# radiusxyz/delay-encryption-in-halo2

Measured on AMD Instinct MI355X. Metric: pallas_msm_mpoints_per_s_at_2^20, higher is better.
Workload: dtype u256; 1 GPU; 1 x MSM(2^20, pallas) + 1 x NTT(2^20, pasta_fp) per step per GPU, uniform scalars, SRS tables resident; configs_index=1, steps_in_flight=4, parallelism=single GPU, attempts=1

## Files before the change

delay-encryption-in-halo2_amd/csrc/msm.cuh:

```cuda
#pragma once
#include <algorithm>
#include <cstdlib>
#include <cstdio>
#include <vector>

#include "ec29.cuh"
#include "internal.hpp"
#include "msm_plan.hpp"

#ifndef MSM_ACC_WAVES_ATTR
#ifdef MSM_ACC_CAP
#define MSM_ACC_WAVES_ATTR __attribute__((amdgpu_waves_per_eu(MSM_ACC_CAP, MSM_ACC_CAP)))
#else
#define MSM_ACC_WAVES_ATTR __attribute__((amdgpu_waves_per_eu(4, 4)))
#endif
#endif
#ifdef MSM_HIST_VGPR64
#define MSM_HIST_ATTR __attribute__((amdgpu_num_vgpr(64)))
#else
#define MSM_HIST_ATTR
#endif

#ifndef MSM_TAIL_PRIO
#define MSM_TAIL_PRIO 0
#endif
FP_DEV void msm_tail_prio() {
#if MSM_TAIL_PRIO > 0
    __builtin_amdgcn_s_setprio(MSM_TAIL_PRIO);
#endif
}

FP_DEV u32 merge2_class(u32 S) { return S <= 2 ? 0u : S <= 4 ? 1u : S <= 8 ? 2u : S <= 64 ? 3u : S <= MERGE2_CHUNK ? 4u : 5u; }

FP_DEV bool fe_is_zero_words(const fe& a) { return (a.v[0] | a.v[1] | a.v[2] | a.v[3] | a.v[4] | a.v[5] | a.v[6] | a.v[7]) == 0; }

template <class FS, class Fn>
FP_DEV void for_each_digit(const fe& mont_scalar, u32 c, u32 w_lo, u32 w_hi, Fn f) {
    if (fe_is_zero_words(mont_scalar)) return;
    fe s = f_from_mont<FS>(mont_scalar);
    u32 bits = 0;
#pragma unroll
    for (int i = 0; i < 8; i++) if (s.v[i]) bits = 32u * i + (32u - (u32)__clz((int)s.v[i]));
    const u32 w_end = min(w_hi, (bits + c - 1) / c + 1);
    const u32 mask = (1u << c) - 1, halfv = 1u << (c - 1);
    u32 carry = 0;
    for (u32 w = 0; w < w_end; w++) {
        u32 raw = (s.v[0] & mask) + carry;
#pragma unroll
        for (int i = 0; i < 7; i++) s.v[i] = (s.v[i] >> c) | (s.v[i + 1] << (32 - c));
        s.v[7] >>= c;
        bool neg = raw > halfv;
        carry = neg ? 1u : 0u;
        u32 mag = neg ? (1u << c) - raw : raw;
        if (mag != 0 && w >= w_lo) f(w, mag - 1, neg);
    }
}

struct DigitStream {
    fe s;
    u32 carry, c, mask, halfv;
    template <class FS>
    FP_DEV void init(const fe& mont_scalar, u32 c_) {
        s = f_from_mont<FS>(mont_scalar);
        c = c_; mask = (1u << c) - 1; halfv = 1u << (c - 1); carry = 0;
    }
    FP_DEV bool exhausted() const { return carry == 0 && fe_is_zero_words(s); }
    FP_DEV void next(u32& bucket, bool& neg) {
        u32 raw = (s.v[0] & mask) + carry;
#pragma unroll
        for (int i = 0; i < 7; i++) s.v[i] = (s.v[i] >> c) | (s.v[i + 1] << (32 - c));
        s.v[7] >>= c;
        neg = raw > halfv;
        carry = neg ? 1u : 0u;
        u32 mag = neg ? (1u << c) - raw : raw;
        bucket = mag - 1;
    }
};

FP_DEV bool wave_value_groups(const fe& s, bool active, u32 lane, u32 max_groups, u32& leader, u32& cnt, u32& rank) {
    unsigned long long rem = __ballot(active);
    leader = lane; cnt = 1; rank = 0;
    for (u32 n = 0; rem; n++) {
        if (n == max_groups) return false;
        const int ld = __ffsll((long long)rem) - 1;
        bool eq = active;
#pragma unroll
        for (int w = 0; w < 8; w++) eq &= s.v[w] == (u32)__shfl((int)s.v[w], ld);
        const unsigned long long m = __ballot(eq);
        if (eq) { leader = (u32)ld; cnt = (u32)__popcll(m); rank = (u32)__popcll(m & ((1ull << lane) - 1)); }
        rem &= ~m;
    }
    return true;
}

template <class FS, bool PACK16>
__global__ __launch_bounds__(MSM_SORT_THREADS) MSM_HIST_ATTR void k_msm_hist(MsmGeom g, const fe* scalars, u32* bh, u32* pc) {
    msm_tail_prio();
    extern __shared__ u32 lhist[];
    const u32 bat = blockIdx.z;
    const u32 w_lo = g.G == 1 ? 0 : blockIdx.y * g.wb, w_hi = g.G == 1 ? g.W : min(g.W, w_lo + g.wb);
    const u32 ng = g.G == 1 ? 1 : w_hi - w_lo, grp0 = g.G == 1 ? 0 : w_lo;
    for (u32 b = threadIdx.x; b < (PACK16 ? ng * g.nb / 2 : ng * g.nb); b += blockDim.x) lhist[b] = 0;
    __syncthreads();
    const fe* sc = scalars + (u64)bat * g.n;
    const u32 per = (g.n + g.slices - 1) / g.slices;
    const u32 beg = blockIdx.x * per, end = min(beg + per, g.n);
    const bool one = g.G == 1;
    for (u32 i0 = beg + threadIdx.x; i0 < end; i0 += 4 * blockDim.x) {
        fe s4[4];
#pragma unroll
        for (int j = 0; j < 4; j++)
            if (i0 + j * blockDim.x < end) s4[j] = f_load(&sc[i0 + j * blockDim.x]);
#pragma unroll
        for (int j = 0; j < 4; j++) {
            const bool valid = i0 + j * blockDim.x < end;
            u32 gl, weight, grank;
            const bool grouped = wave_value_groups(s4[j], valid, threadIdx.x & 63, 4, gl, weight, grank);
            if (!grouped) weight = 1;
            const bool counts = grouped ? valid && (threadIdx.x & 63) == gl : valid;
            if (counts)
                for_each_digit<FS>(s4[j], g.c, w_lo, w_hi, [&](u32 w, u32 bucket, bool) {
                    const u32 slot = (one ? 0u : (w - w_lo) * g.nb) + bucket;
                    if (PACK16) atomicAdd(&lhist[slot >> 1], weight << ((slot & 1u) << 4));
                    else atomicAdd(&lhist[slot], weight);
                });
        }
    }
    __syncthreads();
    const u32 sub = msm_sub_bits(g.c), P = g.nb >> sub;
    for (u32 gi = 0; gi < ng; gi++) {
        const u64 gidx = (u64)bat * g.G + grp0 + gi;
        const u32* lh = lhist + (PACK16 ? gi * g.nb / 2 : gi * g.nb);
        if (PACK16) {
            u32* out = bh + ((gidx * g.slices + blockIdx.x) * g.nb) / 2;
            for (u32 w = threadIdx.x; w < g.nb / 2; w += blockDim.x) out[w] = lh[w];
        } else {
            u32* out = bh + (gidx * g.slices + blockIdx.x) * g.nb;
            for (u32 b = threadIdx.x; b < g.nb; b += blockDim.x) out[b] = lh[b];
        }
        u32* pout = pc + (gidx * g.slices + blockIdx.x) * P;
        const u32 nsub = 1u << sub, lane = threadIdx.x & 63;
        for (u32 q = threadIdx.x >> 6; q < P; q += blockDim.x >> 6) {
            u32 sum = 0;
            if (PACK16) {
                for (u32 w = lane; w < nsub / 2; w += 64) { const u32 x = lh[(q << sub) / 2 + w]; sum += (x & 0xffffu) + (x >> 16); }
            } else {
                for (u32 b = lane; b < nsub; b += 64) sum += lh[(q << sub) + b];
            }
#pragma unroll
            for (int d = 32; d > 0; d >>= 1) sum += __shfl_down(sum, d);
            if (lane == 0) pout[q] = sum;
        }
    }
}

template <bool SRC16>
FP_DEV u32 colscan_one(u32 nb, u32 slices, u32 total_buckets, u32* bh, const unsigned short* src16, u32* count, u32 gb) {
    if (gb >= total_buckets) return 0;
    u32 grp = gb / nb, b = gb - grp * nb;
    u32* col = bh + (u64)grp * slices * nb + b;
    const unsigned short* col16 = SRC16 ? src16 + (u64)grp * slices * nb + b : nullptr;
    u32 run = 0;
    u32 k = 0;
    for (; k + 16 <= slices; k += 16) {
        u32 v[16];
#pragma unroll
        for (int j = 0; j < 16; j++) v[j] = SRC16 ? (u32)col16[(u64)(k + j) * nb] : col[(u64)(k + j) * nb];
#pragma unroll
        for (int j = 0; j < 16; j++) {
            col[(u64)(k + j) * nb] = run;
            run += v[j];
        }
    }
    for (; k < slices; k++) {
        u32 v = SRC16 ? (u32)col16[(u64)k * nb] : col[(u64)k * nb];
        col[(u64)k * nb] = run;
        run += v;
    }
    if (count) count[gb] = run;
    return run;
}
static __global__ __launch_bounds__(SCAN_THREADS) void k_msm_colscan(u32 nb, u32 slices, u32 total_buckets, u32* bh, const unsigned short* bh16, u32* count, u32 blocks_a, u32 P,
                                                                     u32 total_parts, u32* pc, u32* bsum_items, u32* bsum_tasks, u32* merge_counters) {
    msm_tail_prio();
    if (blockIdx.x == 0 && threadIdx.x < MSM_MERGE_COUNTERS) merge_counters[threadIdx.x] = 0;
    if (blockIdx.x >= blocks_a) {
        colscan_one<false>(P, slices, total_parts, pc, nullptr, nullptr, (blockIdx.x - blocks_a) * blockDim.x + threadIdx.x);
        return;
    }
    const u32 gb0 = blockIdx.x * blockDim.x + threadIdx.x;
    const u32 v = bh16 ? colscan_one<true>(nb, slices, total_buckets, bh, bh16, count, gb0) : colscan_one<false>(nb, slices, total_buckets, bh, nullptr, count, gb0);
    u32 si = v, st = v ? 1u : 0u;
#pragma unroll
    for (int d = 32; d > 0; d >>= 1) { si += __shfl_down(si, d); st += __shfl_down(st, d); }
    __shared__ u32 w_i[SCAN_THREADS / 64], w_t[SCAN_THREADS / 64];
    if ((threadIdx.x & 63) == 0) { w_i[threadIdx.x >> 6] = si; w_t[threadIdx.x >> 6] = st; }
    __syncthreads();
    if (threadIdx.x == 0) {
        u32 a = 0, b = 0;
        for (u32 w = 0; w < SCAN_THREADS / 64; w++) { a += w_i[w]; b += w_t[w]; }
        bsum_items[blockIdx.x] = a; bsum_tasks[blockIdx.x] = b;
    }
}

static __global__ __launch_bounds__(SCAN_THREADS) void k_scan_offsets(const u32* cnt, u32 total, const u32* bsum_items, const u32* bsum_tasks, u32 nblocks, u32* geo, u32 resident,
                                                                      u32 lmax, u32 lcap, u32 kmin, u32* off, u32* nrank, u32* rbeg, u32* rend, u32* lists, u32 cap) {
    msm_tail_prio();
    __shared__ u32 s_i[SCAN_THREADS], s_t[SCAN_THREADS];
    __shared__ u32 w4[4][SCAN_THREADS / 64];
    const u32 tid = threadIdx.x, lane = tid & 63, wave = tid >> 6;
    u32 bi = 0, bt = 0, ti = 0;
    for (u32 j = tid; j < nblocks; j += SCAN_THREADS) {
        const u32 a = bsum_items[j];
        ti += a;
        if (j < blockIdx.x) { bi += a; bt += bsum_tasks[j]; }
    }
#pragma unroll
    for (int d = 32; d > 0; d >>= 1) { bi += __shfl_down(bi, d); bt += __shfl_down(bt, d); ti += __shfl_down(ti, d); }
    if (lane == 0) { w4[0][wave] = bi; w4[1][wave] = bt; w4[2][wave] = ti; }
    const u32 idx = blockIdx.x * SCAN_THREADS + tid;
    const u32 vi = idx < total ? cnt[idx] : 0, vt = vi ? 1u : 0u;
    s_i[tid] = vi; s_t[tid] = vt;
    __syncthreads();
    bi = 0; bt = 0; ti = 0;
    for (u32 w = 0; w < SCAN_THREADS / 64; w++) { bi += w4[0][w]; bt += w4[1][w]; ti += w4[2][w]; }
    const u64 M = ti;
    u64 L;
    if (lcap) {
        u64 k = kmin;
        while (M > k * resident * lcap) k += k < 4 ? 1 : 2;
        L = max((u64)4, (M + k * resident - 1) / (k * resident));
    } else {
        const u64 rounds = max((u64)1, (M + (u64)resident * lmax - 1) / ((u64)resident * lmax));
        L = (M + rounds * resident - 1) / (rounds * resident);
        L = min((u64)lmax, max((u64)4, L));
    }
    if (blockIdx.x == 0 && tid == 0) { geo[0] = (u32)L; geo[1] = (u32)M; }
    for (u32 d = 1; d < SCAN_THREADS; d <<= 1) {
        const u32 ai = tid >= d ? s_i[tid - d] : 0, at = tid >= d ? s_t[tid - d] : 0;
        __syncthreads();
        s_i[tid] += ai; s_t[tid] += at;
        __syncthreads();
    }
    const u32 ri = bi + s_i[tid] - vi, rt = bt + s_t[tid] - vt;
    u32 S = 0;
    if (idx < total) {
        off[idx] = ri; nrank[idx] = rt;
        const u32 b0 = (u32)(ri / L) + rt;
        const u32 b1 = vi ? (u32)((ri + vi - 1) / L) + rt + 1 : b0;
        rbeg[idx] = b0;
        rend[idx] = b1;
        S = b1 - b0;
        if (idx + 1 == total) { off[total] = ri + vi; nrank[total] = rt + vt; }
    }
    if (!lists) return;
    u32* counters = geo - MSM_MERGE_COUNTERS;
    const u32 cls = S <= 1 ? 8u : merge2_class(S);
    __shared__ u32 wcnt[5][SCAN_THREADS / 64], cbase[5];
    unsigned long long mine = 0;
    for (u32 c = 0; c < 5; c++) {
        const unsigned long long mask = __ballot(cls == c);
        if (cls == c) mine = mask;
        if (lane == 0) wcnt[c][wave] = (u32)__popcll(mask);
    }
    __syncthreads();
    if (tid < 5) {
        u32 tot = 0;
        for (u32 w = 0; w < SCAN_THREADS / 64; w++) tot += wcnt[tid][w];
        cbase[tid] = tot ? atomicAdd(&counters[tid], tot) : 0u;
    }
    __syncthreads();
    if (cls < 5) {
        u32 pos = cbase[cls] + (u32)__popcll(mine & ((1ull << lane) - 1));
        for (u32 w = 0; w < wave; w++) pos += wcnt[cls][w];
        lists[(size_t)cls * cap + pos] = idx;
    }
    if (cls == 5u) {
        const u32 parts = (S + MERGE2_CHUNK - 1) / MERGE2_CHUNK;
        const u32 slot = atomicAdd(&counters[6], 1u), first = atomicAdd(&counters[5], parts);
        u32* hb = lists + (size_t)6 * cap + 4 * (size_t)slot;
        hb[0] = idx; hb[1] = first; hb[2] = parts; hb[3] = 0;
        for (u32 p = 0; p < parts; p++) {
            lists[(size_t)5 * cap + 2 * (size_t)(first + p)] = slot;
            lists[(size_t)5 * cap + 2 * (size_t)(first + p) + 1] = p;
        }
    }
}

template <class FS>
__global__ __launch_bounds__(MSM_SORT_THREADS) void k_msm_part(MsmGeom g, const fe* scalars, const u32* off, const u32* pc, unsigned long long* pairs, u32 lists) {
    msm_tail_prio();
    extern __shared__ __align__(8) unsigned char part_smem[];
    const u32 bat = blockIdx.z;
    const u32 sub = msm_sub_bits(g.c), P = g.nb >> sub, submask = (1u << sub) - 1;
    const u32 w_lo = g.G == 1 ? 0 : blockIdx.y * g.wb, w_hi = g.G == 1 ? g.W : min(g.W, w_lo + g.wb);
    const u32 ng = g.G == 1 ? 1 : w_hi - w_lo, grp0 = g.G == 1 ? 0 : w_lo;
    const u32 PT = ng * P;
    const bool one = g.G == 1;
    const u32 wave = threadIdx.x >> 6, lane = threadIdx.x & 63, nwaves = blockDim.x >> 6;
    u32* pcur = reinterpret_cast<u32*>(part_smem);
    unsigned char* wbase = part_smem + 4 * lists + (size_t)wave * MSM_PART_WAVE_LDS(lists);
    unsigned long long* stage = reinterpret_cast<unsigned long long*>(wbase);
    u32* lcnt = reinterpret_cast<u32*>(wbase + 512 * 8);
    u32* lbase = lcnt + lists;
    u32* lcur = lbase + lists;
    u32* gbase = lcur + lists;
    unsigned short* stageq = reinterpret_cast<unsigned short*>(gbase + lists);
    for (u32 qq = threadIdx.x; qq < PT; qq += blockDim.x) {
        const u32 gi = qq / P, q = qq - gi * P;
        const u64 gidx = (u64)bat * g.G + grp0 + gi;
        pcur[qq] = off[gidx * g.nb + (q << sub)] + pc[(gidx * g.slices + blockIdx.x) * P + q];
    }
    __syncthreads();
    const fe* sc = scalars + (u64)bat * g.n;
    const u32 per = (g.n + g.slices - 1) / g.slices;
    const u32 beg = blockIdx.x * per, end = min(beg + per, g.n);
    (void)nwaves;
    fe s_next;
    if (beg + wave * 64 + lane < end) s_next = f_load(&sc[beg + wave * 64 + lane]);
    for (u32 i0 = beg + wave * 64; i0 < end; i0 += blockDim.x) {
        const u32 i = i0 + lane;
        const bool have = i < end;
        const fe s_cur = s_next;
        if (i + blockDim.x < end) s_next = f_load(&sc[i + blockDim.x]);
        const bool nonzero = have && !fe_is_zero_words(s_cur);
        const unsigned long long actm = __ballot(nonzero);
        if (actm == 0) continue;
        DigitStream ds;
        if (nonzero) ds.template init<FS>(s_cur, g.c);
        {
            u32 gl, gcnt, grank;
            if (__popcll(actm) > 1 && wave_value_groups(s_cur, nonzero, lane, 4, gl, gcnt, grank)) {
                for (u32 w = 0; w < w_hi; w++) {
                    if (__ballot(nonzero && !ds.exhausted()) == 0) break;
                    u32 bk = 0xffffffffu; bool ng1 = false;
                    if (nonzero) ds.next(bk, ng1);
                    const bool put = nonzero && w >= w_lo && bk != 0xffffffffu;
                    const u32 q = put ? (one ? 0u : (w - w_lo) * P) + (bk >> sub) : 0u;
                    u32 g0 = 0;
                    if (put && lane == gl) g0 = atomicAdd(&pcur[q], gcnt);
                    g0 = (u32)__shfl((int)g0, (int)gl);
                    const u32 tidx = one ? w * g.table_n + i : i;
                    if (put) pairs[g0 + grank] = ((unsigned long long)(bk & submask) << 32) | (tidx | (ng1 ? 0x80000000u : 0u));
                }
                continue;
            }
        }
        for (u32 w0 = 0; w0 < w_hi; w0 += 8) {
            if (__ballot(nonzero && !ds.exhausted()) == 0) break;
            u32 bk[8];
            bool ng8[8];
#pragma unroll
            for (int j = 0; j < 8; j++) {
                bk[j] = 0xffffffffu; ng8[j] = false;
                if (nonzero && w0 + j < w_hi) {
                    ds.next(bk[j], ng8[j]);
                    if (w0 + j < w_lo) bk[j] = 0xffffffffu;
                }
            }
            if (w0 + 8 <= w_lo) continue;
            for (u32 q = lane; q < PT; q += 64) lcnt[q] = 0;
            __builtin_amdgcn_wave_barrier();
#pragma unroll
            for (int j = 0; j < 8; j++)
                if (bk[j] != 0xffffffffu) atomicAdd(&lcnt[(one ? 0u : (w0 + j - w_lo) * P) + (bk[j] >> sub)], 1u);
            __builtin_amdgcn_wave_barrier();
            u32 run = 0;
            for (u32 q0 = 0; q0 < PT; q0 += 64) {
                const u32 q = q0 + lane;
                const u32 v = q < PT ? lcnt[q] : 0;
                u32 x = v;
#pragma unroll
                for (int d = 1; d < 64; d <<= 1) { u32 y = __shfl_up(x, d); if ((int)lane >= d) x += y; }
                if (q < PT) {
                    lbase[q] = run + x - v; lcur[q] = run + x - v;
                    gbase[q] = v ? atomicAdd(&pcur[q], v) : 0u;
                }
                run += __shfl(x, 63);
            }
            __builtin_amdgcn_wave_barrier();
#pragma unroll
            for (int j = 0; j < 8; j++)
                if (bk[j] != 0xffffffffu) {
                    const u32 q = (one ? 0u : (w0 + j - w_lo) * P) + (bk[j] >> sub);
                    const u32 pos = atomicAdd(&lcur[q], 1u);
                    const u32 tidx = one ? (w0 + j) * g.table_n + i : i;
                    stage[pos] = ((unsigned long long)(bk[j] & submask) << 32) | (tidx | (ng8[j] ? 0x80000000u : 0u));
                    stageq[pos] = (unsigned short)q;
                }
            __builtin_amdgcn_wave_barrier();
            for (u32 e = lane; e < run; e += 64) {
                const u32 q = stageq[e];
                pairs[gbase[q] + (e - lbase[q])] = stage[e];
            }
            __builtin_amdgcn_wave_barrier();
        }
    }
}

static __global__ __launch_bounds__(256) void k_msm_bucket(u32 nb, u32 c, u32 slices, const u32* off, const u32* bh, const u32* pc,
                                                          const unsigned long long* pairs, u32* idx_out, u32 per_block) {
    msm_tail_prio();
    __shared__ u32 lcur[512], lfirst[512];
    const u32 sub = msm_sub_bits(c), P = nb >> sub, nsub = 1u << sub;
    const u32 chunks = (slices + per_block - 1) / per_block;
    const u64 gidx = blockIdx.y;
    u32 p, ch;
    if ((P & 7) == 0) {
        u32 xcd = blockIdx.x & 7, j = blockIdx.x >> 3;
        p = xcd + 8 * (j / chunks);
        ch = j % chunks;
    } else {
        p = blockIdx.x / chunks;
        ch = blockIdx.x % chunks;
    }
    const u32 k0 = ch * per_block, k1 = min(k0 + per_block, slices);
    const u32* goff = off + gidx * nb + ((u64)p << sub);
    const u32* rel = bh + (gidx * slices + k0) * nb + ((u64)p << sub);
    for (u32 j = threadIdx.x; j < nsub; j += blockDim.x) { lcur[j] = goff[j] + rel[j]; lfirst[j] = goff[j]; }
    const u32 pbase = goff[0];
    const u32 beg = pbase + pc[(gidx * slices + k0) * P + p];
    const u32 end = k1 < slices ? pbase + pc[(gidx * slices + k1) * P + p] : goff[nsub];
    __syncthreads();
    __shared__ u32 cnt[512], sbase[512], scur[512], wsum[4];
    __shared__ u32 stage[2048];
    __shared__ unsigned short stageq[2048];
    const u32 tid = threadIdx.x, lane = tid & 63, wave = tid >> 6;
    for (u32 r0 = beg; r0 < end; r0 += 2048) {
        const u32 rend = min(r0 + 2048u, end);
        unsigned long long pr[8];
        if (tid < nsub) cnt[tid] = 0;
        if (tid + 256 < nsub) cnt[tid + 256] = 0;
        __syncthreads();
#pragma unroll
        for (int j = 0; j < 8; j++) {
            u32 i = r0 + tid + j * 256;
            pr[j] = i < rend ? pairs[i] : ~0ull;
            const bool v = pr[j] != ~0ull;
            const u32 sb = (u32)(pr[j] >> 32);
            const unsigned long long act = __ballot(v);
            if (act && __ballot(v && sb != (u32)__builtin_amdgcn_readfirstlane((int)sb)) == 0 && ((act & 1ull) != 0)) {
                if (lane == 0) atomicAdd(&cnt[sb], (u32)__popcll(act));
            } else if (v) atomicAdd(&cnt[sb], 1u);
        }
        __syncthreads();
        if (nsub <= 256) {
            u32 v = tid < nsub ? cnt[tid] : 0, x = v;
#pragma unroll
            for (int d = 1; d < 64; d <<= 1) { u32 y = __shfl_up(x, d); if ((int)lane >= d) x += y; }
            if (lane == 63) wsum[wave] = x;
            __syncthreads();
            u32 before = 0;
            for (u32 w = 0; w < wave; w++) before += wsum[w];
            if (tid < nsub) { sbase[tid] = before + x - v; scur[tid] = before + x - v; }
        } else {
            const u32 v0 = cnt[2 * tid], v1 = cnt[2 * tid + 1];
            u32 x = v0 + v1;
#pragma unroll
            for (int d = 1; d < 64; d <<= 1) { u32 y = __shfl_up(x, d); if ((int)lane >= d) x += y; }
            if (lane == 63) wsum[wave] = x;
            __syncthreads();
            u32 before = 0;
            for (u32 w = 0; w < wave; w++) before += wsum[w];
            const u32 e0 = before + x - v0 - v1;
            sbase[2 * tid] = e0; scur[2 * tid] = e0;
            sbase[2 * tid + 1] = e0 + v0; scur[2 * tid + 1] = e0 + v0;
        }
        __syncthreads();
#pragma unroll
        for (int j = 0; j < 8; j++) {
            const bool v = pr[j] != ~0ull;
// ... 126 lines not shown
}

template <class CV>
__global__ __launch_bounds__(128) void k_msm_build_table(const affine_t* std_points, affine_t* table, u32 n, u32 c, u32 rows) {
    typedef typename CV::Base F;
    typedef typename f29_of<typename CV::Base>::type F9;
    u32 i = blockIdx.x * blockDim.x + threadIdx.x;
    if (i >= n) return;
    affine_t p = aff_load(&std_points[i]);
    if (!aff_is_identity(p)) { p.x = f_canon_word<F>(p.x); p.y = f_canon_word<F>(p.y); }
    xyzz_t cur = xyzz_from_affine<F>(p);
    for (u32 w = 0; w < rows; w++) {
        affine_t a = p;
        if (w > 0) {
            for (u32 k = 0; k < c; k++) cur = xyzz_double<F>(cur);
            a = xyzz_to_affine<F>(cur);
        }
        affine_t o;
        if (aff_is_identity(a)) { o.x = f_zero(); o.y = f_zero(); }
        else {
            o.x = f29_to_packed_canon<F9>(f29_from_std<F9>(a.x));
            o.y = f29_to_packed_canon<F9>(f29_from_std<F9>(a.y));
        }
        aff_store(&table[(u64)w * n + i], o);
    }
}

template <class CV>
__global__ void k_jac_to_affine(const jacobian_t* in, affine_t* out, u32 count) {
    typedef typename CV::Base F;
    u32 i = blockIdx.x * blockDim.x + threadIdx.x;
    if (i >= count) return;
    fe x = f_load(&in[i].x), y = f_load(&in[i].y), z = f_load(&in[i].z);
    affine_t a;
    if (f_is_zero(z)) { a.x = f_zero(); a.y = f_zero(); }
    else {
        typedef typename f29_of<F>::type F9;
        fe zi = f29_to_std<F9>(f29_inv_safegcd<F9>(f29_from_std<F9>(z)));
        fe zi2 = f_sqr<F>(zi);
        a.x = f_mul<F>(x, zi2);
        a.y = f_mul<F>(y, f_mul<F>(zi2, zi));
    }
    aff_store(&out[i], a);
}


static_assert(sizeof(xyzz29_rec) == MSM_REC_BYTES, "msm_plan.hpp sizes the record buffers");

static DevBuf dehalo_ctx::* const msm_ws_bufs[MSM_WS_N] = {
    &dehalo_ctx::ws_count, &dehalo_ctx::ws_counters, &dehalo_ctx::ws_bhist, &dehalo_ctx::ws_pcount, &dehalo_ctx::ws_pairs, &dehalo_ctx::ws_off, &dehalo_ctx::ws_records,
    &dehalo_ctx::ws_merge_parts, &dehalo_ctx::ws_merge_lists, &dehalo_ctx::ws_idx, &dehalo_ctx::ws_partial0, &dehalo_ctx::ws_buckets, &dehalo_ctx::ws_contrib, &dehalo_ctx::ws_tree,
    &dehalo_ctx::ws_bred_cnt, &dehalo_ctx::ws_gsums, &dehalo_ctx::ws_bsum};

template <class CV>
int run_msm_t(dehalo_ctx* ctx, const dehalo_bases* bases, const fe* d_scalars, size_t len, size_t batch, jacobian_t* d_out, hipStream_t s) {
    typedef typename CV::Scalar FS;
    if (batch == 0) return 0;
    if (len == 0) {
        HIP_TRY(ctx, hipMemsetAsync(d_out, 0, batch * sizeof(jacobian_t), s));
        return 0;
    }
    MsmTuning tuning = msm_experiment_tuning();
    tuning.sort_block = ctx->msm_sort_block; tuning.acc_block = ctx->msm_acc_block; tuning.acc_points = ctx->msm_acc_points; tuning.acc_waves = ctx->msm_acc_waves;
    tuning.acc_min_layers = ctx->msm_acc_min_layers; tuning.num_cus = ctx->num_cus;
    MsmPlan p;
    if (const char* refused = msm_plan(MsmShape{len, batch, bases->n, bases->c, bases->W, bases->precomp != 0}, tuning, &p)) return dh_fail(ctx, DEHALO_ERR_INVALID, refused);
    const MsmGeom& g = p.g;

    for (u32 i = 0; i < MSM_WS_N; i++) {
        DevBuf& b = ctx->*msm_ws_bufs[i];
        const bool grows = p.ws_bytes[i] > b.cap;
        TRY(dh_ensure(ctx, b, p.ws_bytes[i]));
        if (grows && i == MSM_WS_BRED_CNT) HIP_TRY(ctx, hipMemsetAsync(b.p, 0, b.cap, s));
    }
    const u32 tb = (u32)p.total_buckets;
    u32* count = (u32*)ctx->ws_count.p;
    u32* merge_counters = (u32*)ctx->ws_counters.p;
    u32* geo = merge_counters + MSM_MERGE_COUNTERS;
    u32* off = (u32*)ctx->ws_off.p;
    u32* nrank = (u32*)ctx->ws_records.p;
    u32* rbeg = nrank + (p.total_buckets + 1);
    u32* rend = rbeg + (p.total_buckets + 1);
    u32* merge_lists = (u32*)ctx->ws_merge_lists.p;
    u32* bh = (u32*)ctx->ws_bhist.p;
    unsigned short* bh16 = reinterpret_cast<unsigned short*>(bh + p.total_buckets * (size_t)g.slices);
    u32* pc = (u32*)ctx->ws_pcount.p;
    unsigned long long* pairs = (unsigned long long*)ctx->ws_pairs.p;
    u32* bs_i = (u32*)ctx->ws_bsum.p;
    u32* bs_t = bs_i + p.cs_a;
    u32* idx = (u32*)ctx->ws_idx.p;
    xyzz29_rec* partial0 = (xyzz29_rec*)ctx->ws_partial0.p;
    xyzz29_rec* buckets = (xyzz29_rec*)ctx->ws_buckets.p;
    xyzz29_rec* gsums = (xyzz29_rec*)ctx->ws_gsums.p;

    const void* hist_fn = p.pack16 ? (const void*)k_msm_hist<FS, true> : (const void*)k_msm_hist<FS, false>;
    if (p.lds_hist > 48 * 1024) HIP_TRY(ctx, dh_func_lds(ctx, hist_fn, (int)p.lds_hist));
    const size_t lds_part = dh_co_lds_pad(0, p.lds_part);
    HIP_TRY(ctx, dh_func_lds(ctx, (const void*)k_msm_part<FS>, (int)lds_part));
    const size_t lds_bk = dh_co_lds_pad(p.lds_bucket, 0), lds_m = dh_co_lds_pad(18 * 1024, 0), lds_b = dh_co_lds_pad(41 * 1024, 0);
    TRY(dh_co_lds_attr(ctx, (const void*)k_msm_bucket, lds_bk));
    {
        ScopedTimer t(ctx, s, DEHALO_K_MSM_SORT);
        const dim3 grid(p.sort_grid[0], p.sort_grid[1], p.sort_grid[2]);
        if (p.pack16) k_msm_hist<FS, true><<<grid, p.hist_threads, p.lds_hist, s>>>(g, d_scalars, reinterpret_cast<u32*>(bh16), pc);
        else k_msm_hist<FS, false><<<grid, p.hist_threads, p.lds_hist, s>>>(g, d_scalars, bh, pc);
        k_msm_colscan<<<p.cs_a + p.cs_b, SCAN_THREADS, 0, s>>>(g.nb, g.slices, tb, bh, p.pack16 ? bh16 : nullptr, count, p.cs_a, p.P, (u32)p.total_groups * p.P, pc, bs_i, bs_t, merge_counters);
        k_scan_offsets<<<p.cs_a, SCAN_THREADS, 0, s>>>(count, tb, bs_i, bs_t, p.cs_a, geo, (u32)p.resident, (u32)p.lmax, p.lcap, p.kmin, off, nrank, rbeg, rend,
                                                       merge_lists, p.merge_cap);
        HIP_TRY(ctx, hipGetLastError());
        k_msm_part<FS><<<grid, p.part_threads, lds_part, s>>>(g, d_scalars, off, pc, pairs, p.part_lists);
        k_msm_bucket<<<dim3(p.bucket_grid[0], p.bucket_grid[1]), p.bucket_threads, lds_bk, s>>>(g.nb, g.c, g.slices, off, bh, pc, pairs, idx, p.bslices);
        HIP_TRY(ctx, hipGetLastError());
    }
    {
        ScopedTimer t(ctx, s, DEHALO_K_MSM_ACCUMULATE);
        k_msm_accum0<CV><<<p.acc_grid, p.acc_block, p.acc_lds, s>>>(g, tb, idx, off, nrank, bases->table.p, partial0, geo);
        HIP_TRY(ctx, hipGetLastError());
    }
    {
        ScopedTimer t(ctx, s, DEHALO_K_MSM_REDUCE);
        TRY(dh_co_lds_attr(ctx, (const void*)k_msm_merge2<CV>, lds_m));
        TRY(dh_co_lds_attr(ctx, (const void*)k_msm_bred<CV>, lds_b));
        TRY(msm_stamps_arm(ctx));
        k_msm_merge2<CV><<<MERGE2_GRID, 256, lds_m, s>>>(rbeg, rend, partial0, buckets, merge_counters, merge_lists, p.merge_cap, (xyzz29_rec*)ctx->ws_merge_parts.p, tb);
        const bool fin = g.G == 1;
        k_msm_bred<CV><<<dim3(p.nblk, (u32)p.total_groups), BRED_THREADS, lds_b, s>>>(g.nb, p.bred_bb, buckets, (xyzz29_rec*)ctx->ws_contrib.p, (xyzz29_rec*)ctx->ws_tree.p, (u32*)ctx->ws_bred_cnt.p, gsums,
                                                                                     fin ? d_out : nullptr, fin ? ctx->msm_affine_out : nullptr);
        TRY(msm_stamps_report(ctx, g.nb, (u32)p.total_groups, tb, s));
        if (!fin) k_msm_final<CV><<<g.batch, 256, 0, s>>>(g, gsums, d_out, ctx->msm_affine_out);
        HIP_TRY(ctx, hipGetLastError());
    }
    return 0;
}

template <class CV>
int build_table_t(dehalo_ctx* ctx, dehalo_bases* b, const affine_t* d_std_points, hipStream_t s) {
    u32 rows = b->precomp ? b->W : 1;
    k_msm_build_table<CV><<<(u32)((b->n + 127) / 128), 128, 0, s>>>(d_std_points, b->table.p, (u32)b->n, b->c, rows);
    HIP_TRY(ctx, hipGetLastError());
    return 0;
}

template <class CV>
__global__ __launch_bounds__(64) void k_point_sum(const jacobian_t* in, u32 count, jacobian_t* out) {
    typedef f29_lat<typename f29_of<typename CV::Base>::type> F;
    const u32 lane = threadIdx.x;
    xyzz29 acc = x29_identity();
    for (u32 i = lane; i < count; i += 64) {
        fe z = f_load(&in[i].z);
        if (f_is_zero(z)) continue;
        xyzz29 p;
        f29 z29 = f29_from_std<F>(z);
        p.x = f29_from_std<F>(f_load(&in[i].x));
        p.y = f29_from_std<F>(f_load(&in[i].y));
        p.zz = f29_sqr<F>(z29);
        p.zzz = f29_mul<F>(p.zz, z29);
        acc = x29_add<F>(acc, p);
    }
    acc = x29_group_reduce<F, 64>(acc);
    if (lane == 0) {
        jacobian_t j = x29_to_jacobian_std<F>(acc);
        f_store(&out->x, j.x); f_store(&out->y, j.y); f_store(&out->z, j.z);
    }
}
// ... 21 lines not shown
```

delay-encryption-in-halo2_amd/csrc/msm_plan.hpp:

```cpp
#pragma once
#include <algorithm>
#include <cstddef>
#include <cstdint>
#include <cstdlib>

#include "experiment_env.hpp"

#ifdef __HIPCC__
#define MSM_PLAN_HD __host__ __device__
#else
#define MSM_PLAN_HD
#endif

#define MSM_SORT_THREADS 1024
#define MSM_ACC_THREADS 128
#define MSM_ACC_THREADS_MAX 768
#define MSM_MERGE_COUNTERS 8

#define MERGE2_CHUNK 512

#define MSM_IDX_FIRST 0x40000000u
#define MSM_IDX_MASK 0x3fffffffu

#define SCAN_THREADS 256
// ... 82 lines not shown
    return (256 + c - 1) / c;
}

inline bool msm_table_fits(size_t n, uint32_t W) { return n < (1ull << 30) && (uint64_t)n * W < (1ull << 30); }

struct MsmShape {
    size_t len, batch;
    size_t table_n;
    uint32_t c, W;
    bool precomp;
};

struct MsmTuning {
    int sort_block = 1024, acc_block = 128, acc_points = 48, acc_waves = 3, acc_min_layers = 4;
    int num_cus = 256;
    bool small_slices = true;
    uint32_t hist_threads = 0, part_threads = 0;
    uint32_t bucket_slices = MSM_BUCKET_SLICES;
    bool bucket_fill = true;
    uint32_t acc_lds = 0;
    uint32_t bred_block = 0;
};

inline const MsmTuning& msm_experiment_tuning() {
    static const MsmTuning tuning = [] {
        MsmTuning t;
        auto off = [](const char* e) { return e && e[0] == '0'; };
        auto threads = [](const char* e) { const int v = e ? atoi(e) : 0; return (uint32_t)std::max(0, std::min(MSM_SORT_THREADS, v & ~63)); };
        t.small_slices = !off(DH_EXPERIMENT_ENV("DEHALO_MSM_SMALL_SLICES"));
        t.hist_threads = threads(DH_EXPERIMENT_ENV("DEHALO_MSM_HIST_THREADS"));
        t.part_threads = threads(DH_EXPERIMENT_ENV("DEHALO_MSM_PART_THREADS"));
        if (const char* e = DH_EXPERIMENT_ENV("DEHALO_MSM_BUCKET_SLICES")) { const int v = atoi(e); if (v >= 1 && v <= 16) t.bucket_slices = (uint32_t)v; }
        t.bucket_fill = !off(DH_EXPERIMENT_ENV("DEHALO_MSM_BUCKET_FILL"));
        if (const char* e = DH_EXPERIMENT_ENV("DEHALO_MSM_ACC_LDS")) t.acc_lds = (uint32_t)atoi(e);
        if (const char* e = DH_EXPERIMENT_ENV("DEHALO_MSM_BRED_BLOCK")) { const int v = atoi(e); if (v == 128 || v == 256) t.bred_block = (uint32_t)v; }
        return t;
    }();
    return tuning;
}

enum MsmWs {
    MSM_WS_COUNT, MSM_WS_COUNTERS, MSM_WS_BHIST, MSM_WS_PCOUNT, MSM_WS_PAIRS, MSM_WS_OFF, MSM_WS_RECORDS, MSM_WS_MERGE_PARTS, MSM_WS_MERGE_LISTS, MSM_WS_IDX,
    MSM_WS_PARTIAL0, MSM_WS_BUCKETS, MSM_WS_CONTRIB, MSM_WS_TREE, MSM_WS_BRED_CNT, MSM_WS_GSUMS, MSM_WS_BSUM, MSM_WS_N
};

struct MsmPlan {
    MsmGeom g;
    uint64_t total_groups, total_buckets, Mmax;
    uint32_t P;
    bool pack16;
    uint32_t hist_threads, part_threads, part_lists, sort_grid[3];
    size_t lds_hist, lds_part;
    uint32_t cs_a, cs_b;
    uint32_t bslices, bucket_threads, bucket_grid[2];
    size_t lds_bucket;
    uint32_t lcap, kmin, acc_block, acc_grid, acc_lds;
    uint64_t resident, lmax, lanes_max, nt0_max;
    uint32_t merge_cap, bred_bb, nblk;
    size_t ws_bytes[MSM_WS_N];
};

inline const char* msm_plan(const MsmShape& sh, const MsmTuning& t, MsmPlan* plan) {
    if (sh.c < MSM_WINDOW_MIN) return "msm: window below 4 bits";
    MsmPlan& p = *plan;
    p = MsmPlan{};
    MsmGeom& g = p.g;
    const size_t len = sh.len, batch = sh.batch;
    g.n = (uint32_t)len; g.table_n = (uint32_t)sh.table_n; g.c = sh.c; g.W = sh.W; g.nb = 1u << (g.c - 1);
    g.G = sh.precomp ? 1 : g.W;
    g.batch = (uint32_t)batch;
    g.L0 = 0;
    const uint32_t sort_threads = t.sort_block == 512 ? 512u : 1024u;
    g.slices = (uint32_t)std::min<size_t>(256 * (1024 / sort_threads), std::max<size_t>(1, len / (2 * sort_threads)));
    if (t.small_slices && g.G == 1 && (size_t)g.slices * batch < 128)
        g.slices = (uint32_t)std::max<size_t>(g.slices, std::min<size_t>(std::max<size_t>(1, len / 256), (128 + batch - 1) / batch));
    if ((size_t)g.nb * 4 > 128 * 1024) {
        if (g.G != 1) return "a 17-bit window needs a precomputed table";
        g.slices = (uint32_t)std::max<uint64_t>(g.slices, ((uint64_t)len * g.W + 65534) / 65535);
    }
    p.P = g.nb >> msm_sub_bits(g.c);
    {
        const uint32_t fit = std::min<uint32_t>(std::min<uint32_t>(g.W, 128 / p.P), (128u * 1024 / 4) / g.nb);
        const uint32_t fill = (uint32_t)((uint64_t)g.W * g.slices * batch / 256);
        g.wb = g.G == 1 ? g.W : std::max<uint32_t>(1, std::min<uint32_t>(fit, fill));
    }
    p.total_groups = (uint64_t)batch * g.G;
    p.total_buckets = p.total_groups * g.nb;
    p.Mmax = (uint64_t)batch * len * g.W;
    if (p.Mmax >= (1ull << 32) || p.total_buckets >= (1ull << 31)) return "batch * len * windows too large for one launch";
    const uint64_t tg = p.total_groups, tb = p.total_buckets;

    const uint32_t per_slice = (uint32_t)((len + g.slices - 1) / g.slices);
    p.pack16 = g.nb >= 2 && (uint64_t)per_slice * (g.G == 1 ? g.W : g.wb) <= 65535;
    p.lds_hist = (size_t)g.nb * (p.pack16 ? 2 : 4) * (g.G == 1 ? 1 : g.wb);
    p.hist_threads = t.hist_threads ? t.hist_threads : sort_threads;
    p.part_threads = t.part_threads ? t.part_threads : sort_threads;
    p.part_lists = (g.G == 1 ? p.P : 128u) > 128u ? 256u : 128u;
    p.lds_part = 4 * (size_t)p.part_lists + (size_t)(p.part_threads / 64) * MSM_PART_WAVE_LDS(p.part_lists);
    p.sort_grid[0] = g.slices; p.sort_grid[1] = g.G == 1 ? 1 : (g.G + g.wb - 1) / g.wb; p.sort_grid[2] = (uint32_t)batch;
    p.cs_a = ((uint32_t)tb + SCAN_THREADS - 1) / SCAN_THREADS;
    p.cs_b = ((uint32_t)tg * p.P + SCAN_THREADS - 1) / SCAN_THREADS;
    p.bslices = t.bucket_slices;
    while (t.bucket_fill && p.bslices > 1 && (uint64_t)p.P * ((g.slices + p.bslices - 1) / p.bslices) * tg < (uint64_t)t.num_cus) p.bslices >>= 1;
    p.bucket_threads = MSM_BUCKET_THREADS;
    p.bucket_grid[0] = p.P * ((g.slices + p.bslices - 1) / p.bslices); p.bucket_grid[1] = (uint32_t)tg;
    p.lds_bucket = 22 * 1024;

    p.lcap = (uint32_t)t.acc_points;
    p.kmin = (uint32_t)t.acc_min_layers;
    p.resident = (uint64_t)t.num_cus * 4 * (p.lcap ? 1 : (uint64_t)t.acc_waves) * 64;
    p.lmax = 64 * 4 / (uint64_t)t.acc_waves;
    p.acc_block = t.acc_block == MSM_ACC_THREADS_MAX ? MSM_ACC_THREADS_MAX : MSM_ACC_THREADS;
    if (p.lcap) {
        uint64_t k = 4;
        while (p.Mmax > k * p.resident * p.lcap) k += 2;
        p.lanes_max = k * p.resident + p.acc_block;
    } else {
        const uint64_t rounds_max = std::max<uint64_t>(1, (p.Mmax + p.resident * p.lmax - 1) / (p.resident * p.lmax));
        p.lanes_max = rounds_max * p.resident + p.acc_block;
    }
    p.nt0_max = p.lanes_max + tb;
    p.acc_grid = (uint32_t)((p.lanes_max + p.acc_block - 1) / p.acc_block);
    p.acc_lds = t.acc_lds;

    p.merge_cap = (uint32_t)std::max<uint64_t>(std::min<uint64_t>(tb, p.nt0_max / 2 + 1), 4 * (p.nt0_max / MERGE2_CHUNK + 2));
    const bool bred_forced = t.bred_block && g.nb / t.bred_block <= BRED_FANIN * BRED_FANIN;
    p.bred_bb = bred_forced ? t.bred_block : (g.nb <= 8192 ? 128u : 256u);
    p.nblk = std::max<uint32_t>(1, g.nb / p.bred_bb);

    const size_t REC = MSM_REC_BYTES;
    size_t* ws = p.ws_bytes;
    ws[MSM_WS_COUNT] = tb * 4;
    ws[MSM_WS_COUNTERS] = 64;
    ws[MSM_WS_BHIST] = tb * (size_t)g.slices * 6;
    ws[MSM_WS_PCOUNT] = tg * (size_t)g.slices * p.P * 4;
    ws[MSM_WS_PAIRS] = p.Mmax * 8;
    ws[MSM_WS_OFF] = (tb + 1) * 4;
    ws[MSM_WS_RECORDS] = (tb + 1) * 4 * 3;
    ws[MSM_WS_MERGE_PARTS] = (2 * (p.nt0_max / MERGE2_CHUNK) + 4) * REC;
    ws[MSM_WS_MERGE_LISTS] = (size_t)p.merge_cap * MSM_MERGE_COUNTERS * 4;
    ws[MSM_WS_IDX] = p.Mmax * 4;
    ws[MSM_WS_PARTIAL0] = p.nt0_max * REC;
    ws[MSM_WS_BUCKETS] = tb * REC;
    ws[MSM_WS_CONTRIB] = tg * std::max<size_t>(1, g.nb / BRED_BLOCK_BUCKETS_MIN) * BRED_VMAX * REC;
    ws[MSM_WS_TREE] = tg * 16 * BRED_VMAX * REC;
    ws[MSM_WS_BRED_CNT] = (size_t)tg * BRED_CNT_PER_GROUP * 4;
    ws[MSM_WS_GSUMS] = tg * REC;
    ws[MSM_WS_BSUM] = (size_t)p.cs_a * 2 * sizeof(uint32_t);
    return nullptr;
}
```

Measured before the change: 837.7 Mpoints/s.

## Specialize digit extraction per window size and compact colscan output per bucket chunk

```diff
diff --git a/delay-encryption-in-halo2_amd/csrc/msm.cuh b/delay-encryption-in-halo2_amd/csrc/msm.cuh
--- a/delay-encryption-in-halo2_amd/csrc/msm.cuh
+++ b/delay-encryption-in-halo2_amd/csrc/msm.cuh
@@ -34,13 +34,66 @@
 
 FP_DEV bool fe_is_zero_words(const fe& a) { return (a.v[0] | a.v[1] | a.v[2] | a.v[3] | a.v[4] | a.v[5] | a.v[6] | a.v[7]) == 0; }
 
-template <class FS, class Fn>
+#define MSM_STATIC_WINDOWS(X) X(13) X(15) X(16) X(17)
+
+FP_DEV u32 fe_bit_length(const fe& s) {
+    u32 bits = 0;
+#pragma unroll
+    for (int i = 0; i < 8; i++) if (s.v[i]) bits = 32u * i + (32u - (u32)__clz((int)s.v[i]));
+    return bits;
+}
+template <u32 V> struct u32_c { static constexpr u32 value = V; };
+template <u32 I, u32 N, class F>
+FP_DEV void static_for_while(F&& f) {
+    if constexpr (I < N) { if (f(u32_c<I>{})) static_for_while<I + 1, N>(f); }
+}
+template <u32 C, u32 LO>
+FP_DEV u32 fe_window_at(const fe& s) {
+    constexpr u32 i = LO >> 5, sh = LO & 31;
+    if constexpr (i > 7) return 0;
+    else if constexpr (sh + C <= 32) return (s.v[i] >> sh) & ((1u << C) - 1);
+    else if constexpr (i == 7) return s.v[7] >> sh;
+    else return ((s.v[i] >> sh) | (s.v[i + 1] << (32 - sh))) & ((1u << C) - 1);
+}
+template <u32 K>
+FP_DEV void fe_shr_static(fe& s) {
+    constexpr u32 wq = K >> 5, sh = K & 31;
+    static_for_while<0, 8>([&](auto ic) {
+        constexpr u32 i = decltype(ic)::value;
+        u32 a = 0, b = 0;
+        if constexpr (i + wq < 8) a = s.v[i + wq];
+        if constexpr (i + wq + 1 < 8) b = s.v[i + wq + 1];
+        if constexpr (sh != 0) s.v[i] = (a >> sh) | (b << (32 - sh));
+        else s.v[i] = a;
+        return true;
+    });
+}
+template <u32 C>
+FP_DEV void signed_digit(u32 raw, u32& carry, u32& bucket, bool& neg) {
+    raw += carry;
+    neg = raw > (1u << (C - 1));
+    carry = neg ? 1u : 0u;
+    bucket = (neg ? (1u << C) - raw : raw) - 1;
+}
+
+template <class FS, u32 C, class Fn>
 FP_DEV void for_each_digit(const fe& mont_scalar, u32 c, u32 w_lo, u32 w_hi, Fn f) {
     if (fe_is_zero_words(mont_scalar)) return;
     fe s = f_from_mont<FS>(mont_scalar);
-    u32 bits = 0;
-#pragma unroll
-    for (int i = 0; i < 8; i++) if (s.v[i]) bits = 32u * i + (32u - (u32)__clz((int)s.v[i]));
+    const u32 bits = fe_bit_length(s);
+    if constexpr (C != 0) {
+        const u32 w_end = min(w_hi, (bits + C - 1) / C + 1);
+        u32 carry = 0;
+        static_for_while<0, (256 + C - 1) / C>([&](auto wc) {
+            constexpr u32 w = decltype(wc)::value;
+            if (w >= w_end) return false;
+            u32 bucket; bool neg;
+            signed_digit<C>(fe_window_at<C, C * w>(s), carry, bucket, neg);
+            if (bucket != 0xffffffffu && w >= w_lo) f(w, bucket, neg);
+            return true;
+        });
+        return;
+    }
     const u32 w_end = min(w_hi, (bits + c - 1) / c + 1);
     const u32 mask = (1u << c) - 1, halfv = 1u << (c - 1);
     u32 carry = 0;
@@ -56,6 +109,7 @@
     }
 }
 
+template <u32 C>
 struct DigitStream {
     fe s;
     u32 carry, c, mask, halfv;
@@ -75,11 +129,27 @@
         u32 mag = neg ? (1u << c) - raw : raw;
         bucket = mag - 1;
     }
+    template <u32 W>
+    FP_DEV void digit_at(u32& bucket, bool& neg) {
+        if constexpr (C != 0) signed_digit<C>(fe_window_at<C, C * W>(s), carry, bucket, neg);
+    }
+    FP_DEV void advance() {
+        if constexpr (C != 0) fe_shr_static<8 * C>(s);
+    }
+    FP_DEV bool exhausted_at(u32 w, u32 bits) const { return carry == 0 && C * w >= bits; }
 };
 
 FP_DEV bool wave_value_groups(const fe& s, bool active, u32 lane, u32 max_groups, u32& leader, u32& cnt, u32& rank) {
     unsigned long long rem = __ballot(active);
     leader = lane; cnt = 1; rank = 0;
+    {
+        unsigned long long left = rem;
+        for (u32 n = 0; n < max_groups && left; n++) {
+            const int ld = __ffsll((long long)left) - 1;
+            left &= ~__ballot(active && s.v[0] == (u32)__builtin_amdgcn_readlane((int)s.v[0], ld));
+        }
+        if (left) return false;
+    }
     for (u32 n = 0; rem; n++) {
         if (n == max_groups) return false;
         const int ld = __ffsll((long long)rem) - 1;
@@ -93,7 +163,7 @@
     return true;
 }
 
-template <class FS, bool PACK16>
+template <class FS, bool PACK16, u32 C>
 __global__ __launch_bounds__(MSM_SORT_THREADS) MSM_HIST_ATTR void k_msm_hist(MsmGeom g, const fe* scalars, u32* bh, u32* pc) {
     msm_tail_prio();
     extern __shared__ u32 lhist[];
@@ -119,7 +189,7 @@
             if (!grouped) weight = 1;
             const bool counts = grouped ? valid && (threadIdx.x & 63) == gl : valid;
             if (counts)
-                for_each_digit<FS>(s4[j], g.c, w_lo, w_hi, [&](u32 w, u32 bucket, bool) {
+                for_each_digit<FS, C>(s4[j], g.c, w_lo, w_hi, [&](u32 w, u32 bucket, bool) {
                     const u32 slot = (one ? 0u : (w - w_lo) * g.nb) + bucket;
                     if (PACK16) atomicAdd(&lhist[slot >> 1], weight << ((slot & 1u) << 4));
                     else atomicAdd(&lhist[slot], weight);
@@ -154,18 +224,16 @@
     }
 }
 
-template <bool SRC16>
-FP_DEV u32 colscan_one(u32 nb, u32 slices, u32 total_buckets, u32* bh, const unsigned short* src16, u32* count, u32 gb) {
-    if (gb >= total_buckets) return 0;
+FP_DEV void colscan_inplace(u32 nb, u32 slices, u32 total, u32* tab, u32 gb) {
+    if (gb >= total) return;
     u32 grp = gb / nb, b = gb - grp * nb;
-    u32* col = bh + (u64)grp * slices * nb + b;
-    const unsigned short* col16 = SRC16 ? src16 + (u64)grp * slices * nb + b : nullptr;
+    u32* col = tab + (u64)grp * slices * nb + b;
     u32 run = 0;
     u32 k = 0;
     for (; k + 16 <= slices; k += 16) {
         u32 v[16];
 #pragma unroll
-        for (int j = 0; j < 16; j++) v[j] = SRC16 ? (u32)col16[(u64)(k + j) * nb] : col[(u64)(k + j) * nb];
+        for (int j = 0; j < 16; j++) v[j] = col[(u64)(k + j) * nb];
 #pragma unroll
         for (int j = 0; j < 16; j++) {
             col[(u64)(k + j) * nb] = run;
@@ -173,23 +241,47 @@
         }
     }
     for (; k < slices; k++) {
-        u32 v = SRC16 ? (u32)col16[(u64)k * nb] : col[(u64)k * nb];
+        u32 v = col[(u64)k * nb];
         col[(u64)k * nb] = run;
         run += v;
     }
-    if (count) count[gb] = run;
+}
+template <class T>
+FP_DEV u32 colscan_groups(u32 nb, u32 slices, u32 bslices, u32 pitch, u32 total_buckets, const T* cnt, u32* rel, u32* count, u32 gb) {
+    if (gb >= total_buckets) return 0;
+    const u32 grp = gb / nb, b = gb - grp * nb;
+    const T* col = cnt + (u64)grp * slices * nb + b;
+    u32* out = rel + (u64)grp * pitch * nb + b;
+    u32 run = 0, k = 0, knext = 0;
+    for (; k + 16 <= slices; k += 16) {
+        u32 v[16];
+#pragma unroll
+        for (int j = 0; j < 16; j++) v[j] = (u32)col[(u64)(k + j) * nb];
+#pragma unroll
+        for (int j = 0; j < 16; j++) {
+            if (k + j == knext) { *out = run; out += nb; knext += bslices; }
+            run += v[j];
+        }
+    }
+    for (; k < slices; k++) {
+        const u32 v = (u32)col[(u64)k * nb];
+        if (k == knext) { *out = run; out += nb; knext += bslices; }
+        run += v;
+    }
+    count[gb] = run;
     return run;
 }
-static __global__ __launch_bounds__(SCAN_THREADS) void k_msm_colscan(u32 nb, u32 slices, u32 total_buckets, u32* bh, const unsigned short* bh16, u32* count, u32 blocks_a, u32 P,
-                                                                     u32 total_parts, u32* pc, u32* bsum_items, u32* bsum_tasks, u32* merge_counters) {
+static __global__ __launch_bounds__(SCAN_THREADS) void k_msm_colscan(u32 nb, u32 slices, u32 bslices, u32 pitch, u32 total_buckets, u32* rel, const unsigned short* cnt16, u32* count,
+                                                                     u32 blocks_a, u32 P, u32 total_parts, u32* pc, u32* bsum_items, u32* bsum_tasks, u32* merge_counters) {
     msm_tail_prio();
     if (blockIdx.x == 0 && threadIdx.x < MSM_MERGE_COUNTERS) merge_counters[threadIdx.x] = 0;
     if (blockIdx.x >= blocks_a) {
-        colscan_one<false>(P, slices, total_parts, pc, nullptr, nullptr, (blockIdx.x - blocks_a) * blockDim.x + threadIdx.x);
+        colscan_inplace(P, slices, total_parts, pc, (blockIdx.x - blocks_a) * blockDim.x + threadIdx.x);
         return;
     }
     const u32 gb0 = blockIdx.x * blockDim.x + threadIdx.x;
-    const u32 v = bh16 ? colscan_one<true>(nb, slices, total_buckets, bh, bh16, count, gb0) : colscan_one<false>(nb, slices, total_buckets, bh, nullptr, count, gb0);
+    const u32 v = cnt16 ? colscan_groups(nb, slices, bslices, pitch, total_buckets, cnt16, rel, count, gb0)
+                        : colscan_groups(nb, slices, bslices, pitch, total_buckets, (const u32*)rel, rel, count, gb0);
     u32 si = v, st = v ? 1u : 0u;
 #pragma unroll
     for (int d = 32; d > 0; d >>= 1) { si += __shfl_down(si, d); st += __shfl_down(st, d); }
@@ -287,7 +379,7 @@
     }
 }
 
-template <class FS>
+template <class FS, u32 C>
 __global__ __launch_bounds__(MSM_SORT_THREADS) void k_msm_part(MsmGeom g, const fe* scalars, const u32* off, const u32* pc, unsigned long long* pairs, u32 lists) {
     msm_tail_prio();
     extern __shared__ __align__(8) unsigned char part_smem[];
@@ -326,15 +418,12 @@
         const bool nonzero = have && !fe_is_zero_words(s_cur);
         const unsigned long long actm = __ballot(nonzero);
         if (actm == 0) continue;
-        DigitStream ds;
+        DigitStream<C> ds;
         if (nonzero) ds.template init<FS>(s_cur, g.c);
         {
             u32 gl, gcnt, grank;
             if (__popcll(actm) > 1 && wave_value_groups(s_cur, nonzero, lane, 4, gl, gcnt, grank)) {
-                for (u32 w = 0; w < w_hi; w++) {
-                    if (__ballot(nonzero && !ds.exhausted()) == 0) break;
-                    u32 bk = 0xffffffffu; bool ng1 = false;
-                    if (nonzero) ds.next(bk, ng1);
+                auto place = [&](u32 w, u32 bk, bool ng1) {
                     const bool put = nonzero && w >= w_lo && bk != 0xffffffffu;
                     const u32 q = put ? (one ? 0u : (w - w_lo) * P) + (bk >> sub) : 0u;
                     u32 g0 = 0;
@@ -342,6 +431,24 @@
                     g0 = (u32)__shfl((int)g0, (int)gl);
                     const u32 tidx = one ? w * g.table_n + i : i;
                     if (put) pairs[g0 + grank] = ((unsigned long long)(bk & submask) << 32) | (tidx | (ng1 ? 0x80000000u : 0u));
+                };
+                if constexpr (C != 0) {
+                    const u32 bits = nonzero ? fe_bit_length(ds.s) : 0u;
+                    static_for_while<0, (256 + C - 1) / C>([&](auto wc) {
+                        constexpr u32 w = decltype(wc)::value;
+                        if (w >= w_hi || __ballot(nonzero && !ds.exhausted_at(w, bits)) == 0) return false;
+                        u32 bk = 0xffffffffu; bool ng1 = false;
+                        if (nonzero) ds.template digit_at<w>(bk, ng1);
+                        place(w, bk, ng1);
+                        return true;
+                    });
+                } else {
+                    for (u32 w = 0; w < w_hi; w++) {
+                        if (__ballot(nonzero && !ds.exhausted()) == 0) break;
+                        u32 bk = 0xffffffffu; bool ng1 = false;
+                        if (nonzero) ds.next(bk, ng1);
+                        place(w, bk, ng1);
+                    }
                 }
                 continue;
             }
@@ -350,12 +457,25 @@
             if (__ballot(nonzero && !ds.exhausted()) == 0) break;
             u32 bk[8];
             bool ng8[8];
-#pragma unroll
-            for (int j = 0; j < 8; j++) {
-                bk[j] = 0xffffffffu; ng8[j] = false;
-                if (nonzero && w0 + j < w_hi) {
-                    ds.next(bk[j], ng8[j]);
-                    if (w0 + j < w_lo) bk[j] = 0xffffffffu;
+            if constexpr (C != 0) {
+                static_for_while<0, 8>([&](auto jc) {
+                    constexpr u32 j = decltype(jc)::value;
+                    bk[j] = 0xffffffffu; ng8[j] = false;
+                    if (nonzero && w0 + j < w_hi) {
+                        ds.template digit_at<j>(bk[j], ng8[j]);
+                        if (w0 + j < w_lo) bk[j] = 0xffffffffu;
+                    }
+                    return true;
+                });
+                if (nonzero) ds.advance();
+            } else {
+#pragma unroll
+                for (int j = 0; j < 8; j++) {
+                    bk[j] = 0xffffffffu; ng8[j] = false;
+                    if (nonzero && w0 + j < w_hi) {
+                        ds.next(bk[j], ng8[j]);
+                        if (w0 + j < w_lo) bk[j] = 0xffffffffu;
+                    }
                 }
             }
             if (w0 + 8 <= w_lo) continue;
@@ -399,7 +519,7 @@
 }
 
 static __global__ __launch_bounds__(256) void k_msm_bucket(u32 nb, u32 c, u32 slices, const u32* off, const u32* bh, const u32* pc,
-                                                          const unsigned long long* pairs, u32* idx_out, u32 per_block) {
+                                                          const unsigned long long* pairs, u32* idx_out, u32 per_block, u32 pitch) {
     msm_tail_prio();
     __shared__ u32 lcur[512], lfirst[512];
     const u32 sub = msm_sub_bits(c), P = nb >> sub, nsub = 1u << sub;
@@ -416,7 +536,7 @@
     }
     const u32 k0 = ch * per_block, k1 = min(k0 + per_block, slices);
     const u32* goff = off + gidx * nb + ((u64)p << sub);
-    const u32* rel = bh + (gidx * slices + k0) * nb + ((u64)p << sub);
+    const u32* rel = bh + (gidx * pitch + ch) * nb + ((u64)p << sub);
     for (u32 j = threadIdx.x; j < nsub; j += blockDim.x) { lcur[j] = goff[j] + rel[j]; lfirst[j] = goff[j]; }
     const u32 pbase = goff[0];
     const u32 beg = pbase + pc[(gidx * slices + k0) * P + p];
@@ -649,6 +769,22 @@
     &dehalo_ctx::ws_merge_parts, &dehalo_ctx::ws_merge_lists, &dehalo_ctx::ws_idx, &dehalo_ctx::ws_partial0, &dehalo_ctx::ws_buckets, &dehalo_ctx::ws_contrib, &dehalo_ctx::ws_tree,
     &dehalo_ctx::ws_bred_cnt, &dehalo_ctx::ws_gsums, &dehalo_ctx::ws_bsum};
 
+struct MsmSortKernels {
+    void (*hist)(MsmGeom, const fe*, u32*, u32*);
+    void (*part)(MsmGeom, const fe*, const u32*, const u32*, unsigned long long*, u32);
+};
+template <class FS, u32 C>
+MsmSortKernels msm_sort_kernels_of(bool pack16) { return {pack16 ? k_msm_hist<FS, true, C> : k_msm_hist<FS, false, C>, k_msm_part<FS, C>}; }
+template <class FS>
+MsmSortKernels msm_sort_kernels(u32 c, bool pack16) {
+    switch (c) {
+#define X(W) case W: return msm_sort_kernels_of<FS, W>(pack16);
+        MSM_STATIC_WINDOWS(X)
+#undef X
+        default: return msm_sort_kernels_of<FS, 0>(pack16);
+    }
+}
+
 template <class CV>
 int run_msm_t(dehalo_ctx* ctx, const dehalo_bases* bases, const fe* d_scalars, size_t len, size_t batch, jacobian_t* d_out, hipStream_t s) {
     typedef typename CV::Scalar FS;
@@ -680,7 +816,8 @@
     u32* rend = rbeg + (p.total_buckets + 1);
     u32* merge_lists = (u32*)ctx->ws_merge_lists.p;
     u32* bh = (u32*)ctx->ws_bhist.p;
-    unsigned short* bh16 = reinterpret_cast<unsigned short*>(bh + p.total_buckets * (size_t)g.slices);
+    u32* bcnt = p.pack16 ? bh + p.total_buckets * (size_t)p.bchunks : bh;
+    unsigned short* bh16 = reinterpret_cast<unsigned short*>(bcnt);
     u32* pc = (u32*)ctx->ws_pcount.p;
     unsigned long long* pairs = (unsigned long long*)ctx->ws_pairs.p;
     u32* bs_i = (u32*)ctx->ws_bsum.p;
@@ -690,23 +827,23 @@
     xyzz29_rec* buckets = (xyzz29_rec*)ctx->ws_buckets.p;
     xyzz29_rec* gsums = (xyzz29_rec*)ctx->ws_gsums.p;
 
-    const void* hist_fn = p.pack16 ? (const void*)k_msm_hist<FS, true> : (const void*)k_msm_hist<FS, false>;
-    if (p.lds_hist > 48 * 1024) HIP_TRY(ctx, dh_func_lds(ctx, hist_fn, (int)p.lds_hist));
+    const MsmSortKernels sort_k = msm_sort_kernels<FS>(g.c, p.pack16);
+    if (p.lds_hist > 48 * 1024) HIP_TRY(ctx, dh_func_lds(ctx, (const void*)sort_k.hist, (int)p.lds_hist));
     const size_t lds_part = dh_co_lds_pad(0, p.lds_part);
-    HIP_TRY(ctx, dh_func_lds(ctx, (const void*)k_msm_part<FS>, (int)lds_part));
+    HIP_TRY(ctx, dh_func_lds(ctx, (const void*)sort_k.part, (int)lds_part));
     const size_t lds_bk = dh_co_lds_pad(p.lds_bucket, 0), lds_m = dh_co_lds_pad(18 * 1024, 0), lds_b = dh_co_lds_pad(41 * 1024, 0);
     TRY(dh_co_lds_attr(ctx, (const void*)k_msm_bucket, lds_bk));
     {
         ScopedTimer t(ctx, s, DEHALO_K_MSM_SORT);
         const dim3 grid(p.sort_grid[0], p.sort_grid[1], p.sort_grid[2]);
-        if (p.pack16) k_msm_hist<FS, true><<<grid, p.hist_threads, p.lds_hist, s>>>(g, d_scalars, reinterpret_cast<u32*>(bh16), pc);
-        else k_msm_hist<FS, false><<<grid, p.hist_threads, p.lds_hist, s>>>(g, d_scalars, bh, pc);
-        k_msm_colscan<<<p.cs_a + p.cs_b, SCAN_THREADS, 0, s>>>(g.nb, g.slices, tb, bh, p.pack16 ? bh16 : nullptr, count, p.cs_a, p.P, (u32)p.total_groups * p.P, pc, bs_i, bs_t, merge_counters);
+        sort_k.hist<<<grid, p.hist_threads, p.lds_hist, s>>>(g, d_scalars, bcnt, pc);
+        k_msm_colscan<<<p.cs_a + p.cs_b, SCAN_THREADS, 0, s>>>(g.nb, g.slices, p.bslices, p.bpitch, tb, bh, p.pack16 ? bh16 : nullptr, count, p.cs_a, p.P,
+                                                               (u32)p.total_groups * p.P, pc, bs_i, bs_t, merge_counters);
         k_scan_offsets<<<p.cs_a, SCAN_THREADS, 0, s>>>(count, tb, bs_i, bs_t, p.cs_a, geo, (u32)p.resident, (u32)p.lmax, p.lcap, p.kmin, off, nrank, rbeg, rend,
                                                        merge_lists, p.merge_cap);
         HIP_TRY(ctx, hipGetLastError());
-        k_msm_part<FS><<<grid, p.part_threads, lds_part, s>>>(g, d_scalars, off, pc, pairs, p.part_lists);
-        k_msm_bucket<<<dim3(p.bucket_grid[0], p.bucket_grid[1]), p.bucket_threads, lds_bk, s>>>(g.nb, g.c, g.slices, off, bh, pc, pairs, idx, p.bslices);
+        sort_k.part<<<grid, p.part_threads, lds_part, s>>>(g, d_scalars, off, pc, pairs, p.part_lists);
+        k_msm_bucket<<<dim3(p.bucket_grid[0], p.bucket_grid[1]), p.bucket_threads, lds_bk, s>>>(g.nb, g.c, g.slices, off, bh, pc, pairs, idx, p.bslices, p.bpitch);
         HIP_TRY(ctx, hipGetLastError());
     }
     {
diff --git a/delay-encryption-in-halo2_amd/csrc/msm_plan.hpp b/delay-encryption-in-halo2_amd/csrc/msm_plan.hpp
--- a/delay-encryption-in-halo2_amd/csrc/msm_plan.hpp
+++ b/delay-encryption-in-halo2_amd/csrc/msm_plan.hpp
@@ -158,7 +158,7 @@
     uint32_t hist_threads, part_threads, part_lists, sort_grid[3];
     size_t lds_hist, lds_part;
     uint32_t cs_a, cs_b;
-    uint32_t bslices, bucket_threads, bucket_grid[2];
+    uint32_t bslices, bchunks, bpitch, bucket_threads, bucket_grid[2];
     size_t lds_bucket;
     uint32_t lcap, kmin, acc_block, acc_grid, acc_lds;
     uint64_t resident, lmax, lanes_max, nt0_max;
@@ -208,8 +208,10 @@
     p.cs_b = ((uint32_t)tg * p.P + SCAN_THREADS - 1) / SCAN_THREADS;
     p.bslices = t.bucket_slices;
     while (t.bucket_fill && p.bslices > 1 && (uint64_t)p.P * ((g.slices + p.bslices - 1) / p.bslices) * tg < (uint64_t)t.num_cus) p.bslices >>= 1;
+    p.bchunks = (g.slices + p.bslices - 1) / p.bslices;
+    p.bpitch = p.pack16 ? p.bchunks : g.slices;
     p.bucket_threads = MSM_BUCKET_THREADS;
-    p.bucket_grid[0] = p.P * ((g.slices + p.bslices - 1) / p.bslices); p.bucket_grid[1] = (uint32_t)tg;
+    p.bucket_grid[0] = p.P * p.bchunks; p.bucket_grid[1] = (uint32_t)tg;
     p.lds_bucket = 22 * 1024;
 
     p.lcap = (uint32_t)t.acc_points;
```

After: 837.7 Mpoints/s, median of 2. About the same (+0.0%).
